# mit-han-lab/qserve

Hardware: AMD Instinct MI355X
Metric: decode tokens/sec/GPU Llama-3-8B W4A8KV4 bs=64 (higher is better)
Workload: dtype int8xint4->int32 (MFMA) + fp16; 1 GPU; Llama-3-8B W4A8 per-channel KV4 decode step, bs=64, context 1024->+512 (BASELINE.json configs[1]); global_batch=64, context_start=1030, parallelism=tp1, hipgraph=True, layers=32, launches_per_layer=8

## Files before the change

### qserve_amd/build.py

```python
import argparse
import concurrent.futures as cf
import os
import shutil
import subprocess
import sys

HERE = os.path.dirname(os.path.abspath(__file__))
CSRC = os.path.join(HERE, "csrc")
BUILD = os.path.join(HERE, "_build")
LIB = os.path.join(HERE, "libqserve_amd.so")
SOURCES = ["lib.hip", "gemm_w4a8.hip", "gemm_w4a8_lds.hip", "gemm_w4a8_tiled.hip", "gemm_w4a8_wide.hip", "gemm_w4a8_ring.hip", "gemm_w8a8.hip", "attention.hip", "attention_mfma.hip", "attention_mfma8.hip", "flash_prefill.hip", "append_attention.hip", "append_attention_split.hip", "append_tree.hip", "tree_accept.hip", "sample_rows.hip", "penalize_rows.hip", "ngram_draft.hip", "stop_update.hip", "page_pool.hip", "logprob_rows.hip", "constrain_rows.hip", "lora_rows.hip", "moe_route.hip", "gemm_w4a8_moe.hip", "append_shared.hip", "fused_small.hip", "direct_allreduce.hip"]
ARCH = "gfx950"
FLAGS = ["-O3", "-std=c++17", "-fPIC", f"--offload-arch={ARCH}", "-Wall", "-Wno-unused-function",
         "-Wno-unused-variable", "-Wno-unused-but-set-variable"]


def hipcc():
    exe = shutil.which("hipcc") or "/opt/rocm/bin/hipcc"
    if not os.path.exists(exe):
        raise RuntimeError("hipcc not found (need ROCm >= 7.0 with the gfx950 target)")
    return exe


def _deps_mtime():
    hdrs = [os.path.join(CSRC, f) for f in os.listdir(CSRC) if f.endswith(".h")]
    hdrs.append(os.path.join(os.path.dirname(HERE), "include", "qserve_amd.h"))
    return max(os.path.getmtime(h) for h in hdrs)


def _compile(src, force, extra, build_dir):
    obj = os.path.join(build_dir, src.replace(".hip", ".o"))
    srcp = os.path.join(CSRC, src)
    if (not force and os.path.exists(obj) and os.path.getmtime(obj) >= max(os.path.getmtime(srcp), _deps_mtime())):
        return obj, False
    cmd = [hipcc(), *FLAGS, *extra, "-c", srcp, "-o", obj]
    r = subprocess.run(cmd, capture_output=True, text=True)
    if r.returncode != 0:
        raise RuntimeError(f"hipcc failed for {src}:\n{r.stderr[-4000:]}")
    return obj, True


def build(force=False, verbose=True, extra=(), timing=False):
    build_dir, lib = BUILD, LIB
    if timing:
        build_dir, lib = os.path.join(HERE, "_build_timing"), os.path.join(HERE, "libqserve_amd_timing.so")
        extra = list(extra) + ["-DQS_TIMING"]
    os.makedirs(build_dir, exist_ok=True)
    extra = list(extra) + os.environ.get("QS_EXTRA_HIPCC_FLAGS", "").split()
    with cf.ThreadPoolExecutor(max_workers=min(8, len(SOURCES))) as ex:
        res = list(ex.map(lambda s: _compile(s, force, list(extra), build_dir), SOURCES))
    objs = [o for o, _ in res]
    rebuilt = any(r for _, r in res)
    if rebuilt or not os.path.exists(lib) or force:
        cmd = [hipcc(), "-shared", "-fPIC", f"--offload-arch={ARCH}", "-Wl,--no-undefined", *objs, "-o", lib]
        r = subprocess.run(cmd, capture_output=True, text=True)
        if r.returncode != 0:
            raise RuntimeError(f"link failed:\n{r.stderr[-4000:]}")
        if verbose:
            print(f"[qserve_amd.build] linked {lib}")
    elif verbose:
        print(f"[qserve_amd.build] up to date: {lib}")
    return lib


if __name__ == "__main__":
    ap = argparse.ArgumentParser()
    ap.add_argument("--force", action="store_true")
    ap.add_argument("--debug-asm", action="store_true",
# ... 8 lines not shown
```

### qserve_amd/csrc/fused_small.hip

```cpp
#include "common.h"
#include "row_ops.h"

namespace {

constexpr int TPB = 256;

template <int NT = TPB>
__device__ __forceinline__ float block_reduce(float v, float* sm, int op) {
    v = op == 0 ? wave_sum(v) : wave_max(v);
    const int wave = threadIdx.x >> 6, lane = threadIdx.x & 63;
    __syncthreads();
    if (lane == 0) sm[wave] = v;
    __syncthreads();
    float r = sm[0];
#pragma unroll
    for (int w = 1; w < NT / 64; ++w) r = op == 0 ? r + sm[w] : fmaxf(r, sm[w]);
    return r;
}
template <int NT = TPB>
__device__ __forceinline__ float block_reduce_once(float v, float* sm, int op) {
    v = op == 0 ? wave_sum(v) : wave_max(v);
    const int wave = threadIdx.x >> 6, lane = threadIdx.x & 63;
    if (lane == 0) sm[wave] = v;
    __syncthreads();
// ... 243 lines not shown
                           qs_stream_t stream) {
    QS_REQUIRE(out && input && weight, "rms_norm: null pointer");
    QS_REQUIRE(hidden > 0 && hidden % 8 == 0, "rms_norm: hidden=%d must be a positive multiple of 8", hidden);
    if (num_tokens <= 0) return QS_OK;
    hipLaunchKernelGGL(rms_norm_kernel, dim3(num_tokens), dim3(TPB), 0, (hipStream_t)stream, (_Float16*)out,
                       (const _Float16*)input, (const _Float16*)weight, epsilon, hidden);
    return qs_launch_status("rms_norm");
}

extern "C" int qs_silu_and_mul(void* out, const void* input, int num_tokens, int d, qs_stream_t stream) {
    QS_REQUIRE(out && input, "silu_and_mul: null pointer");
    QS_REQUIRE(d > 0 && d % 8 == 0, "silu_and_mul: d=%d must be a positive multiple of 8", d);
    if (num_tokens <= 0) return QS_OK;
    int chunks = (d + TPB * 8 - 1) / (TPB * 8);
    if (chunks > 16) chunks = 16;
    hipLaunchKernelGGL(silu_and_mul_kernel, dim3(num_tokens, chunks), dim3(TPB), 0, (hipStream_t)stream, (_Float16*)out,
                       (const _Float16*)input, d);
    return qs_launch_status("silu_and_mul");
}

extern "C" int qs_residual_add(void* a, const void* b, int64_t numel, qs_stream_t stream) {
    QS_REQUIRE(a && b, "residual_add: null pointer");
    QS_REQUIRE(numel % 8 == 0, "residual_add: numel must be a multiple of 8");
    if (numel <= 0) return QS_OK;
    const int64_t n8 = numel / 8;
    int blocks = (int)((n8 + TPB - 1) / TPB);
    if (blocks > 2048) blocks = 2048;
    hipLaunchKernelGGL(residual_add_kernel, dim3(blocks), dim3(TPB), 0, (hipStream_t)stream, (_Float16*)a,
                       (const _Float16*)b, n8);
    return qs_launch_status("residual_add");
}

namespace {
__device__ __forceinline__ void argmax_pick(float& bv, int& bi, float v, int i) {
    if (v > bv || (v == bv && i < bi)) {
        bv = v;
        bi = i;
    }
}
template <int MAXC>
__global__ __launch_bounds__(1024) void argmax_rows_kernel(const _Float16* __restrict__ x, int64_t* __restrict__ out,
                                                            int n, int64_t row_stride) {
    const _Float16* row = x + (size_t)blockIdx.x * row_stride;
    const int tid = threadIdx.x, lane = tid & 63, wave = tid >> 6;
    const int nchunk = n >> 3;
    float bv = -INFINITY;
    int bi = 0x7fffffff;
    for (int c0 = 0; c0 < nchunk; c0 += MAXC * 1024) {
        h8 v[MAXC];
#pragma unroll
        for (int c = 0; c < MAXC; ++c) {
            const int ch = c0 + tid + c * 1024;
            v[c] = load8(row + (size_t)(ch < nchunk ? ch : nchunk - 1) * 8);
        }
#pragma unroll
        for (int c = 0; c < MAXC; ++c) {
            const int ch = c0 + tid + c * 1024;
            if (ch < nchunk) {
#pragma unroll
                for (int e = 0; e < 8; ++e) argmax_pick(bv, bi, (float)v[c][e], ch * 8 + e);
            }
        }
    }
    for (int i = (nchunk << 3) + tid; i < n; i += 1024) argmax_pick(bv, bi, (float)row[i], i);
#pragma unroll
    for (int m = 32; m >= 1; m >>= 1) {
        const float ov = __shfl_xor(bv, m, 64);
        const int oi = __shfl_xor(bi, m, 64);
        argmax_pick(bv, bi, ov, oi);
    }
    __shared__ float s_v[16];
    __shared__ int s_i[16];
    if (lane == 0) {
        s_v[wave] = bv;
        s_i[wave] = bi;
    }
    __syncthreads();
    if (wave == 0) {
        bv = lane < 16 ? s_v[lane] : -INFINITY;
        bi = lane < 16 ? s_i[lane] : 0x7fffffff;
#pragma unroll
        for (int m = 8; m >= 1; m >>= 1) {
            const float ov = __shfl_xor(bv, m, 64);
            const int oi = __shfl_xor(bi, m, 64);
            argmax_pick(bv, bi, ov, oi);
        }
        if (lane == 0) out[blockIdx.x] = bi == 0x7fffffff ? 0 : bi;
    }
}
template <int MAXC>
__global__ __launch_bounds__(1024) void argmax_rows_split_kernel(const _Float16* __restrict__ x, int64_t* __restrict__ out,
                                                                  int n, int64_t row_stride,
                                                                  unsigned long long* __restrict__ keys,
                                                                  unsigned* __restrict__ tickets) {
    const int r = blockIdx.x, part = blockIdx.y, nsplit = gridDim.y;
    const _Float16* row = x + (size_t)r * row_stride;
    const int tid = threadIdx.x, lane = tid & 63, wave = tid >> 6;
    const int nchunk = n >> 3;
    const int per = (nchunk + nsplit - 1) / nsplit;
    const int c_lo = part * per, c_hi = min(nchunk, c_lo + per);
    float bv = -INFINITY;
    int bi = 0x7fffffff;
    for (int c0 = c_lo; c0 < c_hi; c0 += MAXC * 1024) {
        h8 v[MAXC];
#pragma unroll
        for (int c = 0; c < MAXC; ++c) {
            const int ch = c0 + tid + c * 1024;
            v[c] = load8(row + (size_t)(ch < c_hi ? ch : c_hi - 1) * 8);
        }
#pragma unroll
        for (int c = 0; c < MAXC; ++c) {
            const int ch = c0 + tid + c * 1024;
            if (ch < c_hi) {
#pragma unroll
                for (int e = 0; e < 8; ++e) argmax_pick(bv, bi, (float)v[c][e], ch * 8 + e);
            }
        }
    }
    if (part == nsplit - 1)
        for (int i = (nchunk << 3) + tid; i < n; i += 1024) argmax_pick(bv, bi, (float)row[i], i);
#pragma unroll
    for (int m = 32; m >= 1; m >>= 1) {
        const float ov = __shfl_xor(bv, m, 64);
        const int oi = __shfl_xor(bi, m, 64);
        argmax_pick(bv, bi, ov, oi);
    }
    __shared__ float s_v[16];
    __shared__ int s_i[16];
    if (lane == 0) {
        s_v[wave] = bv;
        s_i[wave] = bi;
    }
    __syncthreads();
    if (wave != 0) return;
    bv = lane < 16 ? s_v[lane] : -INFINITY;
    bi = lane < 16 ? s_i[lane] : 0x7fffffff;
#pragma unroll
    for (int m = 8; m >= 1; m >>= 1) {
        const float ov = __shfl_xor(bv, m, 64);
        const int oi = __shfl_xor(bi, m, 64);
        argmax_pick(bv, bi, ov, oi);
    }
    if (lane != 0) return;
    u32 u = __builtin_bit_cast(u32, bv);
    u = (u & 0x80000000u) ? ~u : (u | 0x80000000u);
    const unsigned long long key = ((unsigned long long)u << 32) | (0xFFFFFFFFu - (u32)bi);
    const unsigned long long prev = __hip_atomic_fetch_max(keys + r, key, __ATOMIC_RELAXED, __HIP_MEMORY_SCOPE_AGENT);
    asm volatile("s_waitcnt vmcnt(0)" ::"v"((u32)prev), "v"((u32)(prev >> 32)) : "memory");
    const unsigned t = __hip_atomic_fetch_add(tickets + r, 1u, __ATOMIC_RELAXED, __HIP_MEMORY_SCOPE_AGENT);
    if (t != (unsigned)(nsplit - 1)) return;
    const unsigned long long k = __hip_atomic_exchange(keys + r, 0ull, __ATOMIC_RELAXED, __HIP_MEMORY_SCOPE_AGENT);
    __hip_atomic_store(tickets + r, 0u, __ATOMIC_RELAXED, __HIP_MEMORY_SCOPE_AGENT);
    const u32 idx = 0xFFFFFFFFu - (u32)(k & 0xFFFFFFFFu);
    out[r] = idx == 0x7fffffffu ? 0 : (int64_t)idx;
}

struct ArgmaxWs {
    unsigned long long* keys = nullptr;
    unsigned* tickets = nullptr;
    bool tried = false;
};
constexpr int ARGMAX_WS_ROWS = 8192;
ArgmaxWs* argmax_ws(hipStream_t stream) {
    static ArgmaxWs ws[QS_MAX_DEVICES][QS_MAX_STREAM_SLOTS];
    ArgmaxWs& w = ws[qs_device_slot()][qs_scratch_slot(stream)];
    if (!w.tried) {
        hipStreamCaptureStatus cs = hipStreamCaptureStatusNone;
        if (hipStreamIsCapturing(stream, &cs) != hipSuccess || cs != hipStreamCaptureStatusNone) {
            (void)hipGetLastError();
            return nullptr;
        }
        w.tried = true;
        void* a = nullptr;
        if (hipMalloc(&a, ARGMAX_WS_ROWS * 12) == hipSuccess && hipMemset(a, 0, ARGMAX_WS_ROWS * 12) == hipSuccess &&
            hipDeviceSynchronize() == hipSuccess) {
            w.keys = reinterpret_cast<unsigned long long*>(a);
// ... 162 lines not shown
```

### qserve_amd/csrc/attention_mfma.hip

```cpp
#include "attn_host.h"
#include "kv_quant.h"
#include <mutex>
#include <string.h>

namespace {

constexpr int PAGE_TOK = 64;
constexpr int DH = 128;
constexpr int DHB = 64;
constexpr int UT = 32;
constexpr int USB = UT * DHB;
constexpr int NW = attn_plan::DECODE_WAVES_KV4;
constexpr int NWT = NW;
constexpr int QS_ATTNQ_CAP = 4096;
constexpr int QS_ATTNQ_ROW = 4096;
constexpr int SVC = NW - 1;
#ifndef QS_SEQ
#define QS_SEQ(x) asm volatile("" : "+v"(x))
#endif
constexpr int MAXP = 192;

typedef __attribute__((address_space(1))) uint8_t* g_u8;
typedef __attribute__((address_space(1))) uint16_t* g_u16;
__device__ __forceinline__ void wave_quant_store4(_Float16 v0, _Float16 v1, uint8_t* dst_, __half* scale_p_,
// ... 10 lines not shown
        *zero_p = __builtin_bit_cast(uint16_t, p.zero);
    }
}

__device__ __forceinline__ u32 and_or(u32 x, u32 m, u32 c) {
    return (x & m) | c;
}

typedef __attribute__((address_space(3))) const uint8_t* lds_u8;

template <int G, int EXP = 0>
__global__ __launch_bounds__(NWT * 64, 4) void decode_attention_mfma_kernel(
    const _Float16* __restrict__ q, const _Float16* __restrict__ k, const _Float16* __restrict__ v,
    const int64_t* __restrict__ kv_pointers, const int* __restrict__ lengths, _Float16* __restrict__ out,
    int num_heads, int num_kv_heads, int64_t q_stride0, int64_t kv_stride0, int max_blocks, int timestep,
    float rope_base, const float2* __restrict__ rope_tab, int rope_tab_len, int nsplit, float* __restrict__ ws,
    int8_t* __restrict__ qout, __half* __restrict__ qscale, __half* __restrict__ qrowsum, unsigned* __restrict__ qcounters,
    int kflags) {
    constexpr bool PROFILE = (EXP & 64) != 0;
    __shared__ __attribute__((aligned(16))) uint8_t s_kv[2 * NW * 2 * USB];
    __shared__ __attribute__((aligned(16))) _Float16 s_meta[NW][2][4][UT];
    __shared__ __attribute__((aligned(16))) _Float16 s_q[G][DH];
    __shared__ __attribute__((aligned(16))) _Float16 s_qp[16][DH];
    __shared__ __attribute__((aligned(16))) _Float16 s_knew[DH];
    __shared__ __attribute__((aligned(16))) _Float16 s_vnew[DH];
    __shared__ float s_cur[16];
    __shared__ float2 s_qc[16];
    __shared__ float s_m[NW][G], s_l[NW][G];
    __shared__ int s_flag;

    const int tid = threadIdx.x, lane = tid & 63;
    const int wave = __builtin_amdgcn_readfirstlane(tid >> 6);
    const int hkv = blockIdx.x, b = blockIdx.y;
    __shared__ unsigned long long s_stamps[(EXP & 32) ? NWT * 16 : 1];
    auto stamp = [&](int i) {
        if constexpr (EXP & 32) {
            const unsigned long long t = __builtin_amdgcn_s_memtime();
            if (lane == 0) s_stamps[wave * 16 + i] = t;
        }
    };
    if constexpr (EXP & 32) {
        if (lane < 16) s_stamps[wave * 16 + lane] = 0;
    }
    stamp(0);
    if (!(kflags & 2)) {
        const u32 fa = (u32)(uintptr_t)(__attribute__((address_space(3))) void*)(&s_flag);
        if (tid == SVC * 64) asm volatile("ds_write_b32 %0, %1" ::"v"(fa), "v"(0));
        asm volatile("s_waitcnt lgkmcnt(0)\n\ts_barrier");
    }
    const _Float16* qb = q + (size_t)b * q_stride0 + (size_t)hkv * G * DH;
    const _Float16* kb = k + (size_t)b * kv_stride0 + (size_t)hkv * DH;
    const _Float16* vb = v + (size_t)b * kv_stride0 + (size_t)hkv * DH;
    auto uni_ptr = [](const void* x) -> uint64_t {
        return ((uint64_t)(u32)__builtin_amdgcn_readfirstlane((u32)((uint64_t)(uintptr_t)x >> 32)) << 32) |
               (uint64_t)(u32)__builtin_amdgcn_readfirstlane((u32)(uint64_t)(uintptr_t)x);
    };
    const uint64_t qb_s = uni_ptr(qb), kb_s = uni_ptr(kb), vb_s = uni_ptr(vb);
    const int64_t* ktab = kv_pointers + (size_t)b * 2 * max_blocks;
    const int64_t* vtab = ktab + max_blocks;
    const bool spec = (nsplit == 1 || blockIdx.z == 0);
    if (wave == SVC) {
        asm volatile("s_setprio 3");
        if constexpr (!(EXP & 4)) {
            const u32 lane4 = (u32)lane * 4u;
            auto glds4 = [&](uint64_t sb, const _Float16* dst) {
                const u32 ld = __builtin_amdgcn_readfirstlane((u32)(uintptr_t)(__attribute__((address_space(3))) const void*)dst);
                asm volatile("s_mov_b32 m0, %2\n\ts_nop 4\n\tglobal_load_lds_dword %0, %1" ::"v"(lane4), "s"(sb), "s"(ld) : "memory");
            };
#pragma unroll
            for (int h = 0; h < G; ++h) glds4(qb_s + (uint64_t)(h * DH * 2), &s_q[h][0]);
            glds4(kb_s, &s_knew[0]);
            glds4(vb_s, &s_vnew[0]);
        }
        stamp(5);
    }
    int64_t kpage0, vpage0, kpage7, vpage7;
    int len_raw, gen_raw;
    {
        const int p0 = (wave >> 1) < max_blocks ? (wave >> 1) : 0, p7 = ((wave + NW - 1) >> 1) < max_blocks ? ((wave + NW - 1) >> 1) : 0;
        const uint64_t a0 = uni_ptr(ktab + p0), a1 = uni_ptr(vtab + p0), a2 = uni_ptr(ktab + p7), a3 = uni_ptr(vtab + p7);
        const uint64_t a4 = uni_ptr(lengths ? (const void*)(lengths + b) : (const void*)ktab);
        const uint64_t a5 = uni_ptr(qcounters ? (const void*)(qcounters + b) : (const void*)ktab);
// ... 204 lines not shown
    }

    const float2 qc = s_qc[li & (GP - 1)];
    const float qsum = qc.x, nqoff = -qc.y;
    if constexpr (EXP & 32) {
        float probe = nqoff;
        asm volatile("" : "+v"(probe));
        stamp(11);
    }

    u32 c_lo = 0x000F000Fu, c_hi = 0x00F000F0u, c_magic = 0x64006400u;
    asm volatile("" : "+v"(c_lo), "+v"(c_hi), "+v"(c_magic));

    v4f acc[8];
#pragma unroll
    for (int e = 0; e < 8; ++e) acc[e] = (v4f){0.f, 0.f, 0.f, 0.f};
    float m_run = -3.0e38f, l_part = 0.f, corr = 0.f, psum = 0.f;

    constexpr int NS = GP == 4 ? 2 : 4;
    const int tok0 = 16 * (li >> 3) + 4 * tg + (GP == 4 ? 2 * ((li >> 2) & 1) : 0);
    u32 kl0 = (u32)(uintptr_t)(lptr_t)s_kw + (u32)(li * DHB + 16 * tg);
    u32 vl0 = (u32)(uintptr_t)(lptr_t)s_vw + (u32)((4 * tg) * DHB + 4 * li);
    u32 ml0 = (u32)(uintptr_t)(lptr_t)(&s_meta[wave][0][0][0]) + (u32)(2 * tok0);
    asm volatile("" : "+v"(kl0), "+v"(vl0), "+v"(ml0));
    h8 qB[4];
    {
        const lds_u8 ql = (lds_u8)(&s_qp[0][0]) + (li * (DH * 2) + 64 * tg);
#pragma unroll
        for (int w = 0; w < 4; ++w) qB[w] = *(const __attribute__((address_space(3))) h8*)(ql + 16 * w);
    }

    int it = 0;
    int rem = cnt - 1;
    for (int u = u_first; it < cnt; ++it, --rem, u = unit_of(it)) {
        const bool has2 = rem >= 2;
        asm volatile("; QS_LOOP_BEGIN\n\ts_cmp_eq_u32 %0, 0\n\ts_cbranch_scc1 1f\n\ts_waitcnt vmcnt(9)\n\ts_branch 2f\n1:\n\ts_waitcnt vmcnt(3)\n2:"
                     ::"s"(rem) : "memory", "scc");
        if (it < 2) stamp(5 + 2 * it);
        const int slot = it & 1;
        const int valid = min(UT, tl - u * UT);
        const bool full = valid == UT;
        const int u2 = unit_of(it + 2), valid2 = min(UT, tl - u2 * UT);
        int64_t kpage_next = 0, vpage_next = 0;
        if (has2) next_pages(u2 >> 1, kpage_next, vpage_next);
        if constexpr (EXP & 2) {
            if (has2) dma_a(kpage_next, u2 & 1, slot, valid2);
            asm volatile("s_cmp_lt_u32 %0, 2\n\ts_cbranch_scc1 1f\n\ts_waitcnt vmcnt(9)\n\ts_branch 3f\n1:\n\ts_cmp_eq_u32 %0, 0\n\ts_cbranch_scc1 2f\n\t"
                         "s_waitcnt vmcnt(6)\n\ts_branch 3f\n2:\n\ts_waitcnt vmcnt(0)\n3:" ::"s"(rem) : "memory", "scc");
            if (has2) dma_b(vpage_next, u2 & 1, slot, valid2);
            continue;
        }
        const lds_u8 kl = (lds_u8)(kl0 + (u32)(slot * USB));
        const lds_u8 vl = (lds_u8)(vl0 + (u32)(slot * USB));
        const lds_u8 ml = (lds_u8)(ml0 + (u32)(slot * (4 * UT * 2)));
        v4f craw[2];
#pragma unroll
        for (int t = 0; t < 2; ++t) {
            const v4u raw = *(const __attribute__((address_space(3))) v4u*)(kl + 16 * t * DHB);
            v4f c = {nqoff, nqoff, nqoff, nqoff};
#pragma unroll
            for (int w = 0; w < 4; ++w) {
                const u32 x = raw[w], xs = x >> 8;
                const v4u a4 = {and_or(x, c_lo, c_magic), and_or(x, c_hi, c_magic), and_or(xs, c_lo, c_magic),
                                and_or(xs, c_hi, c_magic)};
                c = __builtin_amdgcn_mfma_f32_16x16x32_f16(__builtin_bit_cast(h8, a4), qB[w], c, 0, 0, 0);
            }
            craw[t] = c;
        }
        float sc[NS];
        float m_new;
        {
            float ksf[NS], kzf[NS];
            if constexpr (GP == 4) {
                const h2 ks = *(const __attribute__((address_space(3))) h2*)(ml);
                const h2 kz = *(const __attribute__((address_space(3))) h2*)(ml + UT * 2);
                ksf[0] = (float)ks[0], ksf[1] = (float)ks[1], kzf[0] = (float)kz[0], kzf[1] = (float)kz[1];
            } else {
                const h4 ks = *(const __attribute__((address_space(3))) h4*)(ml);
                const h4 kz = *(const __attribute__((address_space(3))) h4*)(ml + UT * 2);
#pragma unroll
                for (int j = 0; j < 4; ++j) ksf[j] = (float)ks[j], kzf[j] = (float)kz[j];
            }
#pragma unroll
            for (int j = 0; j < NS; ++j) {
                int x;
                if constexpr (GP == 4) {
                    const float c00 = craw[0][j], c02 = craw[0][2 + j], c10 = craw[1][j], c12 = craw[1][2 + j];
                    x = __builtin_bit_cast(int, c00);
                    x = __builtin_amdgcn_update_dpp(x, __builtin_bit_cast(int, c02), 0x114, 0xF, 0x2, false);
                    x = __builtin_amdgcn_update_dpp(x, __builtin_bit_cast(int, c10), 0x118, 0xF, 0x4, false);
                    x = __builtin_amdgcn_update_dpp(x, __builtin_bit_cast(int, c12), 0x11C, 0xF, 0x8, false);
                } else {
                    const float c0 = craw[0][j], c1 = craw[1][j];
                    x = __builtin_amdgcn_update_dpp(__builtin_bit_cast(int, c0), __builtin_bit_cast(int, c1), 0x118, 0xF, 0xC, false);
                }
                sc[j] = (ksf[j] * qk_scale) * (__builtin_bit_cast(float, x) - kzf[j] * qsum);
            }
            if (!full) {
#pragma unroll
                for (int j = 0; j < NS; ++j)
                    if (tok0 + j >= valid) sc[j] = -3.0e38f;
            }
            asm volatile("s_waitcnt lgkmcnt(0)" ::: "memory");
            if (has2) dma_a(kpage_next, u2 & 1, slot, valid2);
            float mx = sc[0];
#pragma unroll
            for (int j = 1; j < NS; ++j) mx = fmaxf(mx, sc[j]);
            if constexpr (GP == 4) asm volatile("s_nop 1\n\tv_max_f32_dpp %0, %0, %0 row_ror:4 row_mask:0xf bank_mask:0xf" : "+v"(mx));
            asm volatile("s_nop 1\n\tv_max_f32_dpp %0, %0, %0 row_ror:8 row_mask:0xf bank_mask:0xf" : "+v"(mx));
            {
                const int xi = __builtin_bit_cast(int, mx);
                const auto r = __builtin_amdgcn_permlane16_swap(xi, xi, false, false);
                mx = fmaxf(__builtin_bit_cast(float, (int)r[0]), __builtin_bit_cast(float, (int)r[1]));
            }
            {
                const int xi = __builtin_bit_cast(int, mx);
                const auto r = __builtin_amdgcn_permlane32_swap(xi, xi, false, false);
                mx = fmaxf(__builtin_bit_cast(float, (int)r[0]), __builtin_bit_cast(float, (int)r[1]));
            }
            m_new = fmaxf(m_run, mx);
            const float alpha = __builtin_amdgcn_exp2f(m_run - m_new);
            m_run = m_new;
            if (__any(alpha != 1.0f)) {
                l_part *= alpha;
                corr *= alpha;
                psum *= alpha;
#pragma unroll
                for (int e = 0; e < 8; ++e) acc[e] *= alpha;
            }
        }
        asm volatile("s_cmp_lt_u32 %0, 2\n\ts_cbranch_scc1 1f\n\ts_waitcnt vmcnt(9)\n\ts_branch 3f\n1:\n\ts_cmp_eq_u32 %0, 0\n\ts_cbranch_scc1 2f\n\t"
                     "s_waitcnt vmcnt(6)\n\ts_branch 3f\n2:\n\ts_waitcnt vmcnt(0)\n3:" ::"s"(rem) : "memory", "scc");
        u32 pbv[4];
        {
            float vsf[NS], vzf[NS];
            if constexpr (GP == 4) {
                const h2 vs = *(const __attribute__((address_space(3))) h2*)(ml + 2 * UT * 2);
                const h2 vz = *(const __attribute__((address_space(3))) h2*)(ml + 3 * UT * 2);
                vsf[0] = (float)vs[0], vsf[1] = (float)vs[1], vzf[0] = (float)vz[0], vzf[1] = (float)vz[1];
            } else {
                const h4 vs = *(const __attribute__((address_space(3))) h4*)(ml + 2 * UT * 2);
                const h4 vz = *(const __attribute__((address_space(3))) h4*)(ml + 3 * UT * 2);
#pragma unroll
                for (int j = 0; j < 4; ++j) vsf[j] = (float)vs[j], vzf[j] = (float)vz[j];
            }
            float pp[NS];
#pragma unroll
            for (int j = 0; j < NS; ++j) {
                const float pe = __builtin_amdgcn_exp2f(sc[j] - m_new);
                l_part += pe;
                float ps = (float)(_Float16)(pe * vsf[j]);
                float pz = ps * vzf[j];
                if (!full && tok0 + j >= valid) {
                    ps = 0.f;
                    pz = 0.f;
                }
                corr += pz;
                psum += ps;
                pp[j] = ps;
            }
            if constexpr (GP == 4) {
                const int pk = (int)pack_h2(pp[0], pp[1]);
                pbv[0] = (u32)pk;
                pbv[1] = (u32)__builtin_amdgcn_update_dpp(0, pk, 0x104, 0xF, 0xF, true);
                pbv[2] = (u32)__builtin_amdgcn_update_dpp(0, pk, 0x108, 0xF, 0xF, true);
                pbv[3] = (u32)__builtin_amdgcn_update_dpp(0, pk, 0x10C, 0xF, 0xF, true);
            } else {
                const int pk0 = (int)pack_h2(pp[0], pp[1]), pk1 = (int)pack_h2(pp[2], pp[3]);
                pbv[0] = (u32)pk0;
                pbv[1] = (u32)pk1;
                pbv[2] = (u32)__builtin_amdgcn_update_dpp(0, pk0, 0x108, 0xF, 0xF, true);
                pbv[3] = (u32)__builtin_amdgcn_update_dpp(0, pk1, 0x108, 0xF, 0xF, true);
            }
        }
        {
            const h8 pB = __builtin_bit_cast(h8, (v4u){pbv[0], pbv[1], pbv[2], pbv[3]});
            u32 raw[8];
#pragma unroll
            for (int jj = 0; jj < 8; ++jj) {
                raw[jj] = *(const __attribute__((address_space(3))) u32*)(vl + (16 * (jj >> 2) + (jj & 3)) * DHB);
            }
#pragma unroll
            for (int bb = 0; bb < 4; ++bb) {
                u32 lo[4], hi[4];
#pragma unroll
                for (int pq = 0; pq < 4; ++pq) {
                    const u32 W = __builtin_amdgcn_perm(raw[2 * pq + 1], raw[2 * pq], 0x0c000c00u | bb | ((4u + bb) << 16));
                    lo[pq] = and_or(W, c_lo, c_magic);
                    hi[pq] = and_or(W, c_hi, c_magic);
                }
                const h8 a_lo = __builtin_bit_cast(h8, (v4u){lo[0], lo[1], lo[2], lo[3]});
                const h8 a_hi = __builtin_bit_cast(h8, (v4u){hi[0], hi[1], hi[2], hi[3]});
                acc[2 * bb] = __builtin_amdgcn_mfma_f32_16x16x32_f16(a_lo, pB, acc[2 * bb], 0, 0, 0);
                acc[2 * bb + 1] = __builtin_amdgcn_mfma_f32_16x16x32_f16(a_hi, pB, acc[2 * bb + 1], 0, 0, 0);
            }
        }
        asm volatile("s_waitcnt lgkmcnt(0) ; QS_LOOP_END" ::: "memory");
        if (it < 2) stamp(6 + 2 * it);
        if (has2) dma_b(vpage_next, u2 & 1, slot, valid2);
    }

    const u32 lid2 = fresh_lane_id();
    const int li2 = lid2 & 15, tg2 = lid2 >> 4, tid2 = wave * 64 + (int)lid2;
    if constexpr (GP == 4) {
        l_part += xor_lane(l_part, lid2, 4);
        corr += xor_lane(corr, lid2, 4);
        psum += xor_lane(psum, lid2, 4);
    }
    l_part += xor_lane(l_part, lid2, 8);
    corr += xor_lane(corr, lid2, 8);
    psum += xor_lane(psum, lid2, 8);
    l_part += xor_lane(l_part, lid2, 16);
    l_part += xor_lane(l_part, lid2, 32);
    corr += xor_lane(corr, lid2, 16);
    corr += xor_lane(corr, lid2, 32);
    psum += xor_lane(psum, lid2, 16);
    psum += xor_lane(psum, lid2, 32);
    if constexpr (!(EXP & 4)) {
        if (wave == SVC && !svc_free) new_token_work();
    }
    asm volatile("s_waitcnt vmcnt(0)" ::: "memory");
    stamp(12);
    __syncthreads();
    stamp(13);
    constexpr int OS = DH + 4;
    float (*s_o)[G][OS] = reinterpret_cast<float (*)[G][OS]>(&s_kv[0]);
    static_assert(sizeof(float) * NW * G * OS <= sizeof(s_kv), "merge area must fit the page buffers");
    if (li2 < G) {
#pragma unroll
        for (int e = 0; e < 8; ++e)
#pragma unroll
            for (int r = 0; r < 4; ++r)
                s_o[wave][li2][8 * (4 * tg2 + r) + e] = ((e & 1) ? acc[e][r] * 0.0625f : acc[e][r]) - (corr + ((e & 1) ? 64.f : 1024.f) * psum);
        if (tg2 == 0) {
            s_m[wave][li2] = m_run;
            s_l[wave][li2] = l_part;
        }
    }
    __syncthreads();
    stamp(14);
    for (int o = tid2; o < G * DH; o += NWT * 64) {
        const int h = o / DH, d = o % DH;
        float M = z == 0 ? s_cur[h] : -3.0e38f;
#pragma unroll
        for (int w = 0; w < NW; ++w) M = fmaxf(M, s_m[w][h]);
        const float pc = z == 0 ? __builtin_amdgcn_exp2f(s_cur[h] - M) : 0.f;
        float num = pc * (float)((EXP & 4) ? vb[d] : s_vnew[d]), den = pc;
#pragma unroll
        for (int w = 0; w < NW; ++w) {
            const float f = __builtin_amdgcn_exp2f(s_m[w][h] - M);
            num += f * s_o[w][h][d];
            den += f * s_l[w][h];
        }
        if (nsplit == 1) {
            const _Float16 res = (_Float16)(num / (den + 1.e-6f));
            if (qout) reinterpret_cast<_Float16*>(&s_meta[0][0][0])[o] = res;
            else out[((size_t)b * num_heads + (size_t)hkv * G + h) * DH + d] = res;
        } else {
            float* pw = ws + ((((size_t)b * num_kv_heads + hkv) * nsplit + z) * G + h) * (DH + 2);
            pw[d] = num;
            if (d == 0) {
                pw[DH] = M * 0.6931471805599453f;
                pw[DH + 1] = den;
            }
        }
    }
    if (nsplit == 1 && qout) {
        __syncthreads();
        const int hidden = num_heads * DH;
        const unsigned tag = (unsigned)gen_raw + 1u;
        if (tid2 < G * 16) {
            const v4u x = reinterpret_cast<const v4u*>(&s_meta[0][0][0])[tid2];
            *reinterpret_cast<v4u*>(out + ((size_t)b * num_heads + (size_t)hkv * G) * DH + tid2 * 8) = x;
        }
        v2u* const xrow = reinterpret_cast<v2u*>(qcounters + QS_ATTNQ_CAP) + (size_t)b * (QS_ATTNQ_ROW / 2);
        const int own_lo = (num_kv_heads - 1) * G * DH;
        if ((G == 4 || G == 8) && !(kflags & 1024)) {
            float* const sm = reinterpret_cast<float*>(&s_kv[0]);
            v4u* const gran = reinterpret_cast<v4u*>(xrow);
            if (wave == 0) {
                const int ln = (int)lid2;
                float amax = 0.f, s0 = 0.f, s1 = 0.f;
                {
                    const h8 vv = __builtin_bit_cast(h8, reinterpret_cast<const v4u*>(&s_meta[0][0][0])[ln]);
#pragma unroll
                    for (int j = 0; j < 8; ++j) {
                        const float f = (float)vv[j];
                        s0 += f;
                        QS_SEQ(s0);
                        amax = fmaxf(amax, fabsf(f));
                    }
                }
                if (G == 8) {
                    const h8 vv = __builtin_bit_cast(h8, reinterpret_cast<const v4u*>(&s_meta[0][0][0])[64 + ln]);
#pragma unroll
                    for (int j = 0; j < 8; ++j) {
                        const float f = (float)vv[j];
                        s1 += f;
                        QS_SEQ(s1);
                        amax = fmaxf(amax, fabsf(f));
                    }
                }
                amax = wave_max(amax);
                s0 = wave_sum(s0);
                if (G == 8) s1 = wave_sum(s1);
                v4u mine = {__builtin_bit_cast(u32, amax), __builtin_bit_cast(u32, s0), __builtin_bit_cast(u32, s1), tag};
                if (ln == 0 && !((kflags & 64) && b == 0 && hkv == 0) && !(kflags & 512)) {
                    v4u* const dst = gran + hkv;
                    asm volatile("global_store_dwordx4 %0, %1, off sc0 sc1" ::"v"(dst), "v"(mine) : "memory");
                }
                const __amdgpu_buffer_rsrc_t grs = __builtin_amdgcn_make_buffer_rsrc(gran, 0, num_kv_heads * 16, 0x00020000);
                const bool peer = ln < num_kv_heads && ln != hkv;
                const u32 goff = ln < num_kv_heads ? (u32)ln * 16u : 0xFFFFFF00u;
                const int spin_cap = (kflags & 256) ? 1 : (kflags & 64) ? 4096 : QS_SPIN_CAP;
                int polls = 0;
                v4u g;
                for (;;) {
                    g = __builtin_amdgcn_raw_buffer_load_b128(grs, goff, 0, 17);
                    if (!__builtin_amdgcn_ballot_w64(peer && g.w != tag)) break;
                    if (++polls >= spin_cap) {
                        if (ln == 0 && !(kflags & 256))
                            atomicOr(qcounters + QS_ATTNQ_CAP + (size_t)QS_ATTNQ_CAP * QS_ATTNQ_ROW, QS_ERR_ATTN_HANDOVER);
                        break;
                    }
                    __builtin_amdgcn_s_sleep(1);
                }
                if (ln == hkv) g = mine;
                const u32 gx = g.x, gy = g.y, gz = g.z;
                float am = ln < num_kv_heads ? __builtin_bit_cast(float, gx) : 0.f;
                am = wave_max(am);
                float bs;
                if (G == 4) {
                    bs = ln < num_kv_heads ? __builtin_bit_cast(float, gy) : -0.0f;
                } else {
                    const int src = (ln >> 1) < num_kv_heads ? (ln >> 1) : 0;
                    const int yv = __builtin_amdgcn_ds_bpermute(4 * src, (int)gy), zv = __builtin_amdgcn_ds_bpermute(4 * src, (int)gz);
                    bs = (ln >> 1) < num_kv_heads ? __builtin_bit_cast(float, (ln & 1) ? zv : yv) : -0.0f;
                }
                const float tot = wave_sum(bs);
                if (ln == 0) {
                    sm[0] = am;
                    sm[1] = tot;
                }
            }
            __syncthreads();
            const float r = sm[0];
            if (tid2 < G * 16) {
                const h8 vv = __builtin_bit_cast(h8, reinterpret_cast<const v4u*>(&s_meta[0][0][0])[tid2]);
                float f[8];
#pragma unroll
                for (int j = 0; j < 8; ++j) f[j] = (float)vv[j];
                qs_store_q8(qout + (size_t)b * hidden + (size_t)hkv * G * DH + tid2 * 8, f, 127.0f / r);
            }
            if (hkv == num_kv_heads - 1 && tid2 == 0) {
                qscale[b] = __float2half_rn(r / 127.0f);
                if (qrowsum) qrowsum[b] = __float2half_rn(sm[1]);
                qcounters[b] = tag;
            }
        } else if (hkv != num_kv_heads - 1) {
// ... 59 lines not shown
                    sm[tid2 >> 6] = amax;
                    sm[4 + (tid2 >> 6)] = sum[0];
                    sm[8 + (tid2 >> 6)] = sum[1];
                }
            }
            __syncthreads();
            if (tid2 < 256) {
                float r = sm[0];
#pragma unroll
                for (int w = 1; w < 4; ++w) r = fmaxf(r, sm[w]);
                float s2 = 0.f;
                if (qrowsum && tid2 < 64) s2 = wave_sum(tid2 < (hidden + 511) / 512 ? sm[4 + tid2] : -0.0f);
                if (tid2 == 0) {
                    qscale[b] = __float2half_rn(r / 127.0f);
                    if (qrowsum) qrowsum[b] = __float2half_rn(s2);
                    qcounters[b] = tag;
                }
                const float mul = 127.0f / r;
#pragma unroll
                for (int c = 0; c < 2; ++c) {
                    const int i = (c * 256 + tid2) * 8;
                    if (i < hidden) {
                        const h8 vv = __builtin_bit_cast(h8, raw[c]);
                        float f[8];
#pragma unroll
                        for (int j = 0; j < 8; ++j) f[j] = (float)vv[j];
                        qs_store_q8(qout + (size_t)b * hidden + i, f, mul);
                    }
                }
            }
        }
    }
    stamp(15);
    if constexpr (EXP & 32) {
        if (lane < 16)
            reinterpret_cast<unsigned long long*>(ws)[(((size_t)b * gridDim.x + hkv) * NWT + wave) * 16 + lane] = s_stamps[wave * 16 + lane];
    }
}

__global__ __launch_bounds__(DH) void decode_attention_merge_kernel(const float* __restrict__ ws, _Float16* __restrict__ out,
                                                                    int num_heads, int num_kv_heads, int G, int nsplit) {
    const int b = blockIdx.y, hq = blockIdx.x, d = threadIdx.x;
    const int hkv = hq / G, h = hq % G;
    const float* base = ws + (((size_t)b * num_kv_heads + hkv) * nsplit * G + h) * (DH + 2);
    const size_t zs = (size_t)G * (DH + 2);
    float M = -3.0e38f;
    for (int zz = 0; zz < nsplit; ++zz) M = fmaxf(M, base[zz * zs + DH]);
    float num = 0.f, den = 0.f;
    for (int zz = 0; zz < nsplit; ++zz) {
        const float f = __expf(base[zz * zs + DH] - M);
        num += f * base[zz * zs + d];
        den += f * base[zz * zs + DH + 1];
    }
    out[((size_t)b * num_heads + hq) * DH + d] = (_Float16)(num / (den + 1.e-6f));
}

__global__ void rope_table_kernel(float2* tab, int max_pos, float base) {
    const int i = blockIdx.x * blockDim.x + threadIdx.x;
    if (i >= max_pos * 64) return;
    const RopeCS cs = rope_coef_any(i & 63, i >> 6, base, DH, tab);
    tab[i] = make_float2(cs.c, cs.s);
}

struct RopeTable {
    float2* tab = nullptr;
    int len = 0;
    float base = 0.f;
};
constexpr int ROPE_SLOTS = 8;
// ... 294 lines not shown
    const float2* tab = qs_rope_table(base, max_pos, st, &tab_len);
    if (base < 0.f && !tab) return QS_EINVAL;
    const int blocks = (int)(grid.x * grid.y);
    const size_t per_split = attn_plan::decode_split_bytes(blocks, G);
    int nsplit = plan.nsplit > 1 ? attn_plan::fit_splits(plan.nsplit, per_split, qs_split_workspace_capacity(), attn_plan::NO_SPLIT_CAP) : 1;
    float* ws = nsplit > 1 ? qs_split_workspace(per_split * nsplit, st) : nullptr;
    if (!ws) nsplit = 1;
    grid.z = nsplit;
    int8_t* qout = nullptr;
    __half *qscale = nullptr, *qsum = nullptr;
    unsigned* qcnt = nullptr;
    const bool sum_order_ok = !(quant && qs_get_row_sum_order() && quant->qsum);
    if (quant && sum_order_ok && nsplit == 1 && H * DH <= 4096 && (qcnt = qs_attn_quant_counters(st, (int)grid.y))) {
        qout = quant->qout;
        qscale = reinterpret_cast<__half*>(quant->qscale);
        qsum = reinterpret_cast<__half*>(quant->qsum);
        *fused = true;
        if (g_inject_fault & 2) kflags |= 64, g_inject_fault &= ~2;
    }
#define QS_LAUNCH_GP(KERNEL)                                                                                                      \
    hipLaunchKernelGGL((KERNEL), grid, dim3(NWT * 64), 0, st, q, k, v, kvp, len, out, H, Hkv, qs, kvs, mb, timestep, base, tab, tab_len, \
                       nsplit, ws, qout, qscale, qsum, qcnt, kflags)
#define QS_LAUNCH_G(GG)                                                \
    if (base < 0.f) QS_LAUNCH_GP((decode_attention_mfma_kernel<GG, 64>));  \
    else QS_LAUNCH_GP(decode_attention_mfma_kernel<GG>)
#define QS_LAUNCH_EXP(E)                                                                                              \
    case E:                                                                                                            \
        hipLaunchKernelGGL((decode_attention_mfma_kernel<4, E>), grid, dim3(NWT * 64), 0, st, q, k, v, kvp, len, out, H,  \
                           Hkv, qs, kvs, mb, timestep, base, tab, tab_len, nsplit, ws, qout, qscale, qsum, qcnt, kflags); \
        return qs_launch_status("single_query_attention")
#ifdef QS_TIMING
    if (const char* e = getenv("QS_ATTN_KFLAGS")) kflags = atoi(e);
    if (exp_flags & 32) {
        ws = qs_split_workspace((size_t)blocks * NWT * 16 * 8, st);
        if (!ws) exp_flags = 0;
    }
    if (G == 4 && exp_flags > 0 && nsplit == 1) {
        switch (exp_flags) {
            QS_LAUNCH_EXP(1);
            QS_LAUNCH_EXP(2);
            QS_LAUNCH_EXP(4);
            QS_LAUNCH_EXP(6);
            QS_LAUNCH_EXP(32);
            default: break;
        }
    }
#endif
    switch (G) {
        case 1: QS_LAUNCH_G(1); break;
        case 2: QS_LAUNCH_G(2); break;
        case 3: QS_LAUNCH_G(3); break;
        case 4: QS_LAUNCH_G(4); break;
        case 5: QS_LAUNCH_G(5); break;
        case 6: QS_LAUNCH_G(6); break;
        case 7: QS_LAUNCH_G(7); break;
        case 8: QS_LAUNCH_G(8); break;
        default:
            qs_set_error("single_query_attention: num_heads/num_kv_heads = %d not in 1..8", G);
            return QS_ENOSUP;
    }
#undef QS_LAUNCH_G
#undef QS_LAUNCH_GP
    if (nsplit > 1)
        hipLaunchKernelGGL(decode_attention_merge_kernel, dim3(H, grid.y), dim3(DH), 0, st, ws, out, H, Hkv, G, nsplit);
    return qs_launch_status("single_query_attention");
}
```

Before: 23090 tokens/s.

## Rewrite row argmax as packed fp16 max pass then index search

Restructures the argmax kernels into two phases. The first finds the row maximum with packed v_pk_max_f16 over the loaded registers, with no per-element index tracking. The second rescans only in waves that hold the maximum to find the smallest matching index, merged with an LDS atomicMin. Separately, the build enables kernarg preloading for fused_small and the ring GEMM unit to trim kernel launch prologue latency. NaN handling and tie-breaking semantics change slightly, and the rescan reloads from memory when the row exceeds the register chunk.

```diff
diff --git a/qserve_amd/build.py b/qserve_amd/build.py
--- a/qserve_amd/build.py
+++ b/qserve_amd/build.py
@@ -13,6 +13,8 @@
 ARCH = "gfx950"
 FLAGS = ["-O3", "-std=c++17", "-fPIC", f"--offload-arch={ARCH}", "-Wall", "-Wno-unused-function",
          "-Wno-unused-variable", "-Wno-unused-but-set-variable"]
+UNIT_FLAGS = {"fused_small.hip": ["-mllvm", "-amdgpu-kernarg-preload-count=16"],
+              "gemm_w4a8_ring.hip": ["-mllvm", "-amdgpu-kernarg-preload-count=16"]}
 
 
 def hipcc():
@@ -33,7 +35,7 @@
     srcp = os.path.join(CSRC, src)
     if (not force and os.path.exists(obj) and os.path.getmtime(obj) >= max(os.path.getmtime(srcp), _deps_mtime())):
         return obj, False
-    cmd = [hipcc(), *FLAGS, *extra, "-c", srcp, "-o", obj]
+    cmd = [hipcc(), *FLAGS, *UNIT_FLAGS.get(src, []), *extra, "-c", srcp, "-o", obj]
     r = subprocess.run(cmd, capture_output=True, text=True)
     if r.returncode != 0:
         raise RuntimeError(f"hipcc failed for {src}:\n{r.stderr[-4000:]}")
diff --git a/qserve_amd/csrc/fused_small.hip b/qserve_amd/csrc/fused_small.hip
--- a/qserve_amd/csrc/fused_small.hip
+++ b/qserve_amd/csrc/fused_small.hip
@@ -299,61 +299,79 @@
 }
 
 namespace {
-__device__ __forceinline__ void argmax_pick(float& bv, int& bi, float v, int i) {
-    if (v > bv || (v == bv && i < bi)) {
-        bv = v;
-        bi = i;
-    }
+__device__ __forceinline__ h2 pk_max(h2 a, h2 b) {
+    h2 r;
+    asm("v_pk_max_f16 %0, %1, %2" : "=v"(r) : "v"(a), "v"(b));
+    return r;
+}
+template <int MAXC>
+__device__ __forceinline__ void block_argmax(const _Float16* __restrict__ row, int c_lo, int c_hi, int t_lo, int n, float& bv,
+                                             int& bi) {
+    const int tid = threadIdx.x, lane = tid & 63, wave = tid >> 6;
+    __shared__ float s_v[16];
+    __shared__ int s_i;
+    const _Float16 ninf = (_Float16)(-INFINITY);
+    h2 pm = {ninf, ninf};
+    h8 v[MAXC];
+    for (int c0 = c_lo; c0 < c_hi; c0 += MAXC * 1024) {
+#pragma unroll
+        for (int c = 0; c < MAXC; ++c) v[c] = load8(row + (size_t)min(c0 + tid + c * 1024, c_hi - 1) * 8);
+#pragma unroll
+        for (int c = 0; c < MAXC; ++c) {
+            const h2 *d = reinterpret_cast<const h2*>(&v[c]);
+            pm = pk_max(pm, pk_max(pk_max(d[0], d[1]), pk_max(d[2], d[3])));
+        }
+    }
+    float tm = fmaxf((float)pm[0], (float)pm[1]);
+    const int ti = t_lo + tid;
+    float tv = -INFINITY;
+    if (ti < n) {
+        tv = (float)row[ti];
+        tm = fmaxf(tm, tv);
+    }
+    const float wm = wave_max(tm);
+    if (tid == 0) s_i = 0x7fffffff;
+    if (lane == 0) s_v[wave] = wm;
+    __syncthreads();
+    float bm = s_v[0];
+#pragma unroll
+    for (int w = 1; w < 16; ++w) bm = fmaxf(bm, s_v[w]);
+    if (!(bm == bm)) bm = -INFINITY;
+    if (__any(tm == bm)) {
+        int idx = (ti < n && tv == bm) ? ti : 0x7fffffff;
+        if (c_hi - c_lo > MAXC * 1024) {
+            for (int ch = c_lo + tid; ch < c_hi; ch += 1024) {
+                const h8 x = load8(row + (size_t)ch * 8);
+                int hit = 0x7fffffff;
+#pragma unroll
+                for (int e = 7; e >= 0; --e)
+                    if ((float)x[e] == bm) hit = ch * 8 + e;
+                idx = min(idx, hit);
+            }
+        } else if (c_hi > c_lo) {
+#pragma unroll
+            for (int c = MAXC - 1; c >= 0; --c) {
+                const int ch = min(c_lo + tid + c * 1024, c_hi - 1);
+#pragma unroll
+                for (int e = 7; e >= 0; --e)
+                    if ((float)v[c][e] == bm) idx = ch * 8 + e;
+            }
+        }
+#pragma unroll
+        for (int m = 32; m >= 1; m >>= 1) idx = min(idx, __shfl_xor(idx, m, 64));
+        if (lane == 0 && idx != 0x7fffffff) atomicMin(&s_i, idx);
+    }
+    __syncthreads();
+    bv = bm;
+    bi = s_i;
 }
 template <int MAXC>
 __global__ __launch_bounds__(1024) void argmax_rows_kernel(const _Float16* __restrict__ x, int64_t* __restrict__ out,
                                                             int n, int64_t row_stride) {
-    const _Float16* row = x + (size_t)blockIdx.x * row_stride;
-    const int tid = threadIdx.x, lane = tid & 63, wave = tid >> 6;
-    const int nchunk = n >> 3;
-    float bv = -INFINITY;
-    int bi = 0x7fffffff;
-    for (int c0 = 0; c0 < nchunk; c0 += MAXC * 1024) {
-        h8 v[MAXC];
-#pragma unroll
-        for (int c = 0; c < MAXC; ++c) {
-            const int ch = c0 + tid + c * 1024;
-            v[c] = load8(row + (size_t)(ch < nchunk ? ch : nchunk - 1) * 8);
-        }
-#pragma unroll
-        for (int c = 0; c < MAXC; ++c) {
-            const int ch = c0 + tid + c * 1024;
-            if (ch < nchunk) {
-#pragma unroll
-                for (int e = 0; e < 8; ++e) argmax_pick(bv, bi, (float)v[c][e], ch * 8 + e);
-            }
-        }
-    }
-    for (int i = (nchunk << 3) + tid; i < n; i += 1024) argmax_pick(bv, bi, (float)row[i], i);
-#pragma unroll
-    for (int m = 32; m >= 1; m >>= 1) {
-        const float ov = __shfl_xor(bv, m, 64);
-        const int oi = __shfl_xor(bi, m, 64);
-        argmax_pick(bv, bi, ov, oi);
-    }
-    __shared__ float s_v[16];
-    __shared__ int s_i[16];
-    if (lane == 0) {
-        s_v[wave] = bv;
-        s_i[wave] = bi;
-    }
-    __syncthreads();
-    if (wave == 0) {
-        bv = lane < 16 ? s_v[lane] : -INFINITY;
-        bi = lane < 16 ? s_i[lane] : 0x7fffffff;
-#pragma unroll
-        for (int m = 8; m >= 1; m >>= 1) {
-            const float ov = __shfl_xor(bv, m, 64);
-            const int oi = __shfl_xor(bi, m, 64);
-            argmax_pick(bv, bi, ov, oi);
-        }
-        if (lane == 0) out[blockIdx.x] = bi == 0x7fffffff ? 0 : bi;
-    }
+    float bv;
+    int bi;
+    block_argmax<MAXC>(x + (size_t)blockIdx.x * row_stride, 0, n >> 3, n & ~7, n, bv, bi);
+    if (threadIdx.x == 0) out[blockIdx.x] = bi == 0x7fffffff ? 0 : bi;
 }
 template <int MAXC>
 __global__ __launch_bounds__(1024) void argmax_rows_split_kernel(const _Float16* __restrict__ x, int64_t* __restrict__ out,
@@ -361,54 +379,14 @@
                                                                   unsigned long long* __restrict__ keys,
                                                                   unsigned* __restrict__ tickets) {
     const int r = blockIdx.x, part = blockIdx.y, nsplit = gridDim.y;
-    const _Float16* row = x + (size_t)r * row_stride;
-    const int tid = threadIdx.x, lane = tid & 63, wave = tid >> 6;
     const int nchunk = n >> 3;
     const int per = (nchunk + nsplit - 1) / nsplit;
     const int c_lo = part * per, c_hi = min(nchunk, c_lo + per);
-    float bv = -INFINITY;
-    int bi = 0x7fffffff;
-    for (int c0 = c_lo; c0 < c_hi; c0 += MAXC * 1024) {
-        h8 v[MAXC];
-#pragma unroll
-        for (int c = 0; c < MAXC; ++c) {
-            const int ch = c0 + tid + c * 1024;
-            v[c] = load8(row + (size_t)(ch < c_hi ? ch : c_hi - 1) * 8);
-        }
-#pragma unroll
-        for (int c = 0; c < MAXC; ++c) {
-            const int ch = c0 + tid + c * 1024;
-            if (ch < c_hi) {
-#pragma unroll
-                for (int e = 0; e < 8; ++e) argmax_pick(bv, bi, (float)v[c][e], ch * 8 + e);
-            }
-        }
-    }
-    if (part == nsplit - 1)
-        for (int i = (nchunk << 3) + tid; i < n; i += 1024) argmax_pick(bv, bi, (float)row[i], i);
-#pragma unroll
-    for (int m = 32; m >= 1; m >>= 1) {
-        const float ov = __shfl_xor(bv, m, 64);
-        const int oi = __shfl_xor(bi, m, 64);
-        argmax_pick(bv, bi, ov, oi);
-    }
-    __shared__ float s_v[16];
-    __shared__ int s_i[16];
-    if (lane == 0) {
-        s_v[wave] = bv;
-        s_i[wave] = bi;
-    }
-    __syncthreads();
-    if (wave != 0) return;
-    bv = lane < 16 ? s_v[lane] : -INFINITY;
-    bi = lane < 16 ? s_i[lane] : 0x7fffffff;
-#pragma unroll
-    for (int m = 8; m >= 1; m >>= 1) {
-        const float ov = __shfl_xor(bv, m, 64);
-        const int oi = __shfl_xor(bi, m, 64);
-        argmax_pick(bv, bi, ov, oi);
-    }
-    if (lane != 0) return;
+    float bv;
+    int bi;
+    block_argmax<MAXC>(x + (size_t)r * row_stride, c_lo, c_hi, part == nsplit - 1 ? (n & ~7) : n, n, bv, bi);
+    if (threadIdx.x != 0) return;
+    if (bv == 0.f) bv = 0.f;
     u32 u = __builtin_bit_cast(u32, bv);
     u = (u & 0x80000000u) ? ~u : (u | 0x80000000u);
     const unsigned long long key = ((unsigned long long)u << 32) | (0xFFFFFFFFu - (u32)bi);
```

New measurement: 23150 tokens/s (median of 4 runs). About the same (+0.3%).

## Drop pre-merge barrier by staging per-wave partials in ring slots; faster lane reductions

Applied to the files above, without the earlier changes.

Expands the profiling stamp infrastructure with segment timers and realtime stamps, which are compiled only in timing builds. In the default path, the final cross-lane reductions now use DPP shifts and permlane16/32 swaps instead of xor_lane shuffles. Each wave writes its output partials into its own two ring slots in the KV buffer with vectorized stores, which removes the __syncthreads that used to sit before the merge-area writes. The risk is that a wave's slots might still be read by in-flight DMA or by another wave, and the shift-based reductions must produce the same sums as the xor pattern.

```diff
diff --git a/qserve_amd/csrc/attention_mfma.hip b/qserve_amd/csrc/attention_mfma.hip
--- a/qserve_amd/csrc/attention_mfma.hip
+++ b/qserve_amd/csrc/attention_mfma.hip
@@ -66,22 +66,58 @@
     const int tid = threadIdx.x, lane = tid & 63;
     const int wave = __builtin_amdgcn_readfirstlane(tid >> 6);
     const int hkv = blockIdx.x, b = blockIdx.y;
-    __shared__ unsigned long long s_stamps[(EXP & 32) ? NWT * 16 : 1];
+    constexpr int TS = 32;
+    constexpr bool DETAIL = (EXP & 48) == 48;
+    constexpr unsigned LIGHT = (1u << 0) | (1u << 2) | (1u << 5) | (1u << 12) | (1u << 14) | (1u << 15) | (1u << 22) | (1u << 25) |
+                               (1u << 26) | (1u << 28);
+    __shared__ unsigned long long s_stamps[(EXP & 32) ? NWT * TS : 1];
     auto stamp = [&](int i) {
         if constexpr (EXP & 32) {
-            const unsigned long long t = __builtin_amdgcn_s_memtime();
-            if (lane == 0) s_stamps[wave * 16 + i] = t;
+            if ((DETAIL || ((LIGHT >> i) & 1u)) && !(kflags & 2048)) {
+                unsigned long long t;
+                asm volatile("s_memtime %0\n\ts_waitcnt lgkmcnt(0)" : "=s"(t)::"memory");
+                if (lane == 0) s_stamps[wave * TS + i] = t;
+            }
         }
     };
     if constexpr (EXP & 32) {
-        if (lane < 16) s_stamps[wave * 16 + lane] = 0;
-    }
+        if (lane < TS) s_stamps[wave * TS + lane] = 0;
+    }
+    unsigned long long t_seg = 0, seg[6] = {0, 0, 0, 0, 0, 0};
+    auto tick = [&]() {
+        if constexpr ((EXP & 48) == 48) asm volatile("s_memtime %0\n\ts_waitcnt lgkmcnt(0)" : "=s"(t_seg)::"memory");
+    };
+    auto segment = [&](int k) {
+        if constexpr ((EXP & 48) == 48) {
+            const unsigned long long t0 = t_seg;
+            tick();
+            seg[k] += t_seg - t0;
+        }
+    };
+    auto mark = [&](int i) {
+        if constexpr ((EXP & 48) == 48) {
+            if (lane == 0) s_stamps[wave * TS + i] = t_seg;
+        } else {
+            stamp(i);
+        }
+    };
     stamp(0);
+    auto stamp_realtime = [&](int i) {
+        if constexpr (EXP & 32) {
+            if ((DETAIL || ((LIGHT >> i) & 1u)) && !(kflags & 2048)) {
+                unsigned long long t;
+                asm volatile("s_memrealtime %0\n\ts_waitcnt lgkmcnt(0)" : "=s"(t)::"memory");
+                if (lane == 0) s_stamps[wave * TS + i] = t;
+            }
+        }
+    };
+    stamp_realtime(27);
     if (!(kflags & 2)) {
         const u32 fa = (u32)(uintptr_t)(__attribute__((address_space(3))) void*)(&s_flag);
         if (tid == SVC * 64) asm volatile("ds_write_b32 %0, %1" ::"v"(fa), "v"(0));
         asm volatile("s_waitcnt lgkmcnt(0)\n\ts_barrier");
     }
+    stamp(9);
     const _Float16* qb = q + (size_t)b * q_stride0 + (size_t)hkv * G * DH;
     const _Float16* kb = k + (size_t)b * kv_stride0 + (size_t)hkv * DH;
     const _Float16* vb = v + (size_t)b * kv_stride0 + (size_t)hkv * DH;
@@ -352,11 +388,15 @@
 
     int it = 0;
     int rem = cnt - 1;
+    tick();
     for (int u = u_first; it < cnt; ++it, --rem, u = unit_of(it)) {
         const bool has2 = rem >= 2;
+        segment(5);
         asm volatile("; QS_LOOP_BEGIN\n\ts_cmp_eq_u32 %0, 0\n\ts_cbranch_scc1 1f\n\ts_waitcnt vmcnt(9)\n\ts_branch 2f\n1:\n\ts_waitcnt vmcnt(3)\n2:"
                      ::"s"(rem) : "memory", "scc");
-        if (it < 2) stamp(5 + 2 * it);
+        segment(0);
+        if (it < 2) mark(5 + 2 * it);
+        if (rem == 0) mark(23);
         const int slot = it & 1;
         const int valid = min(UT, tl - u * UT);
         const bool full = valid == UT;
@@ -422,6 +462,7 @@
                     if (tok0 + j >= valid) sc[j] = -3.0e38f;
             }
             asm volatile("s_waitcnt lgkmcnt(0)" ::: "memory");
+            segment(1);
             if (has2) dma_a(kpage_next, u2 & 1, slot, valid2);
             float mx = sc[0];
 #pragma unroll
@@ -449,8 +490,11 @@
                 for (int e = 0; e < 8; ++e) acc[e] *= alpha;
             }
         }
+        segment(2);
         asm volatile("s_cmp_lt_u32 %0, 2\n\ts_cbranch_scc1 1f\n\ts_waitcnt vmcnt(9)\n\ts_branch 3f\n1:\n\ts_cmp_eq_u32 %0, 0\n\ts_cbranch_scc1 2f\n\t"
                      "s_waitcnt vmcnt(6)\n\ts_branch 3f\n2:\n\ts_waitcnt vmcnt(0)\n3:" ::"s"(rem) : "memory", "scc");
+        segment(3);
+        if (rem == 0) mark(22);
         u32 pbv[4];
         {
             float vsf[NS], vzf[NS];
@@ -516,47 +560,66 @@
             }
         }
         asm volatile("s_waitcnt lgkmcnt(0) ; QS_LOOP_END" ::: "memory");
-        if (it < 2) stamp(6 + 2 * it);
+        segment(4);
+        if (it < 2) mark(6 + 2 * it);
         if (has2) dma_b(vpage_next, u2 & 1, slot, valid2);
     }
 
+    if constexpr (EXP & 32) {
+        if (lane == 0) {
+#pragma unroll
+            for (int j = 0; j < 6; ++j) s_stamps[wave * TS + 16 + j] = seg[j];
+            s_stamps[wave * TS + 24] = (unsigned long long)cnt;
+        }
+    }
     const u32 lid2 = fresh_lane_id();
     const int li2 = lid2 & 15, tg2 = lid2 >> 4, tid2 = wave * 64 + (int)lid2;
+    auto add_shl4 = [](float x) { return x + __builtin_bit_cast(float, __builtin_amdgcn_update_dpp(0, __builtin_bit_cast(int, x), 0x104, 0xF, 0xF, true)); };
+    auto add_shl8 = [](float x) { return x + __builtin_bit_cast(float, __builtin_amdgcn_update_dpp(0, __builtin_bit_cast(int, x), 0x108, 0xF, 0xF, true)); };
+    auto add_xor16 = [](float x) {
+        const int xi = __builtin_bit_cast(int, x);
+        const auto r = __builtin_amdgcn_permlane16_swap(xi, xi, false, false);
+        return __builtin_bit_cast(float, (int)r[0]) + __builtin_bit_cast(float, (int)r[1]);
+    };
+    auto add_xor32 = [](float x) {
+        const int xi = __builtin_bit_cast(int, x);
+        const auto r = __builtin_amdgcn_permlane32_swap(xi, xi, false, false);
+        return __builtin_bit_cast(float, (int)r[0]) + __builtin_bit_cast(float, (int)r[1]);
+    };
     if constexpr (GP == 4) {
-        l_part += xor_lane(l_part, lid2, 4);
-        corr += xor_lane(corr, lid2, 4);
-        psum += xor_lane(psum, lid2, 4);
-    }
-    l_part += xor_lane(l_part, lid2, 8);
-    corr += xor_lane(corr, lid2, 8);
-    psum += xor_lane(psum, lid2, 8);
-    l_part += xor_lane(l_part, lid2, 16);
-    l_part += xor_lane(l_part, lid2, 32);
-    corr += xor_lane(corr, lid2, 16);
-    corr += xor_lane(corr, lid2, 32);
-    psum += xor_lane(psum, lid2, 16);
-    psum += xor_lane(psum, lid2, 32);
+        l_part = add_shl4(l_part);
+        corr = add_shl4(corr);
+        psum = add_shl4(psum);
+    }
+    l_part = add_xor32(add_xor16(add_shl8(l_part)));
+    corr = add_xor32(add_xor16(add_shl8(corr)));
+    psum = add_xor32(add_xor16(add_shl8(psum)));
     if constexpr (!(EXP & 4)) {
         if (wave == SVC && !svc_free) new_token_work();
     }
     asm volatile("s_waitcnt vmcnt(0)" ::: "memory");
     stamp(12);
-    __syncthreads();
-    stamp(13);
     constexpr int OS = DH + 4;
-    float (*s_o)[G][OS] = reinterpret_cast<float (*)[G][OS]>(&s_kv[0]);
-    static_assert(sizeof(float) * NW * G * OS <= sizeof(s_kv), "merge area must fit the page buffers");
+    static_assert(sizeof(float) * 4 * OS <= 2 * USB && G <= 8, "four heads' partials must fit a wave's two ring slots");
+    auto part = [&](int w, int h) -> float* {
+        return reinterpret_cast<float*>(s_kv + ((h >> 2) * NW + w) * (2 * USB)) + (h & 3) * OS;
+    };
     if (li2 < G) {
-#pragma unroll
-        for (int e = 0; e < 8; ++e)
-#pragma unroll
-            for (int r = 0; r < 4; ++r)
-                s_o[wave][li2][8 * (4 * tg2 + r) + e] = ((e & 1) ? acc[e][r] * 0.0625f : acc[e][r]) - (corr + ((e & 1) ? 64.f : 1024.f) * psum);
+        float* const po = part(wave, li2) + 32 * tg2;
+#pragma unroll
+        for (int r = 0; r < 4; ++r) {
+            float x[8];
+#pragma unroll
+            for (int e = 0; e < 8; ++e) x[e] = ((e & 1) ? acc[e][r] * 0.0625f : acc[e][r]) - (corr + ((e & 1) ? 64.f : 1024.f) * psum);
+            *reinterpret_cast<v4f*>(po + 8 * r) = (v4f){x[0], x[1], x[2], x[3]};
+            *reinterpret_cast<v4f*>(po + 8 * r + 4) = (v4f){x[4], x[5], x[6], x[7]};
+        }
         if (tg2 == 0) {
             s_m[wave][li2] = m_run;
             s_l[wave][li2] = l_part;
         }
     }
+    stamp(13);
     __syncthreads();
     stamp(14);
     for (int o = tid2; o < G * DH; o += NWT * 64) {
@@ -569,7 +632,7 @@
 #pragma unroll
         for (int w = 0; w < NW; ++w) {
             const float f = __builtin_amdgcn_exp2f(s_m[w][h] - M);
-            num += f * s_o[w][h][d];
+            num += f * part(w, h)[d];
             den += f * s_l[w][h];
         }
         if (nsplit == 1) {
@@ -585,6 +648,7 @@
             }
         }
     }
+    stamp(25);
     if (nsplit == 1 && qout) {
         __syncthreads();
         const int hidden = num_heads * DH;
@@ -645,6 +709,7 @@
                     }
                     __builtin_amdgcn_s_sleep(1);
                 }
+                stamp(26);
                 if (ln == hkv) g = mine;
                 const u32 gx = g.x, gy = g.y, gz = g.z;
                 float am = ln < num_kv_heads ? __builtin_bit_cast(float, gx) : 0.f;
@@ -770,9 +835,10 @@
         }
     }
     stamp(15);
+    stamp_realtime(28);
     if constexpr (EXP & 32) {
-        if (lane < 16)
-            reinterpret_cast<unsigned long long*>(ws)[(((size_t)b * gridDim.x + hkv) * NWT + wave) * 16 + lane] = s_stamps[wave * 16 + lane];
+        if (lane < TS)
+            reinterpret_cast<unsigned long long*>(ws)[(((size_t)b * gridDim.x + hkv) * NWT + wave) * TS + lane] = s_stamps[wave * TS + lane];
     }
 }
 
@@ -1133,7 +1199,7 @@
 #ifdef QS_TIMING
     if (const char* e = getenv("QS_ATTN_KFLAGS")) kflags = atoi(e);
     if (exp_flags & 32) {
-        ws = qs_split_workspace((size_t)blocks * NWT * 16 * 8, st);
+        ws = qs_split_workspace((size_t)blocks * NWT * 32 * 8, st);
         if (!ws) exp_flags = 0;
     }
     if (G == 4 && exp_flags > 0 && nsplit == 1) {
@@ -1143,6 +1209,7 @@
             QS_LAUNCH_EXP(4);
             QS_LAUNCH_EXP(6);
             QS_LAUNCH_EXP(32);
+            QS_LAUNCH_EXP(48);
             default: break;
         }
     }
```

Result: no change. 22810 tokens/s before, 22870 tokens/s after (median of 6 runs) (+0.3%).
